# thangvubk/SoftGroup

Measured on AMD Instinct MI355X. Metric: scans/sec ScanNet-v2-like inference (softgroup_scannet.yaml, full forward_test), higher is better.
Workload: dtype f32

## Files before the change

include/softgroup_hip.h:

```cpp
#ifndef SOFTGROUP_HIP_H
#define SOFTGROUP_HIP_H

#include <stddef.h>
#include <stdint.h>

#ifdef __cplusplus
extern "C" {
#endif

typedef void *sg_stream_t;

#define SG_OK 0
#define SG_ERR_ARG (-1)
#define SG_ERR_WORKSPACE (-2)
#define SG_ERR_LAUNCH (-3)
#define SG_ERR_UNSUPPORTED (-4)

#define SG_BALLQUERY_MAX_NEIGHBORS 1000
#define SG_OCTREE_NUM_NODES 585
#define SG_OCTREE_NUM_LEAVES 512
#define SG_LISTS_SORTED 1
#define SG_LISTS_RADIUS 2

int sg_version(void);
const char *sg_last_error(void);
int sg_device_info(char *name_host, int name_cap, int *num_cu_host, int *clock_khz_host);

int sg_stream_release(sg_stream_t stream);
int sg_stream_create(sg_stream_t *stream_out);
int sg_stream_destroy(sg_stream_t stream);
int sg_stream_create_priority(sg_stream_t *stream_out, int level);

int sg_voxelize_idx_host(const int64_t *coords_host, int n, int ncol, int mode,
                         int32_t *input_map_host, int32_t *num_voxels_host,
                         int32_t *max_active_host);
int sg_voxelize_idx_fill_host(const int64_t *coords_host, int n, int ncol, int mode,
                              const int32_t *input_map_host, int num_voxels, int max_active,
                              int64_t *out_coords_host, int32_t *out_map_host);
size_t sg_voxelize_idx_workspace_bytes(int n);
int sg_voxelize_idx_build(const int64_t *coords, int n, int ncol, int mode, int32_t *input_map,
                          int32_t *meta, void *ws, size_t ws_bytes, sg_stream_t stream);
int sg_voxelize_idx_fill(const int64_t *coords, int n, int ncol, int mode,
                         const int32_t *input_map, int num_voxels, int max_active,
                         int64_t *out_coords, int32_t *out_map, void *ws, size_t ws_bytes,
                         sg_stream_t stream);

int sg_voxelize_fp(const float *feats, const int32_t *rules, int num_voxels, int max_active,
                   int channels, int average, float *out, sg_stream_t stream);
int sg_voxelize_bp(const float *d_out, const int32_t *rules, int num_voxels, int max_active,
                   int channels, int average, float *d_feats, sg_stream_t stream);

size_t sg_ballquery_workspace_bytes(int n);
int sg_ballquery_build_grid(const float *xyz, const int32_t *batch_idxs, int n, float radius,
                            void *ws, size_t ws_bytes, sg_stream_t stream);
int sg_ballquery_count(const float *xyz, const int32_t *batch_idxs, int n, float radius,
                       int32_t *start_len, int32_t *meta, void *ws, size_t ws_bytes,
                       sg_stream_t stream);
int sg_ballquery_fill(const float *xyz, const int32_t *batch_idxs, int n, float radius,
                      const int32_t *start_len, int32_t *idx, void *ws, size_t ws_bytes,
                      sg_stream_t stream);
size_t sg_scan_workspace_bytes(int n);
int sg_exclusive_scan_startlen(int32_t *start_len, int n, int32_t *meta, void *ws,
                               size_t ws_bytes, sg_stream_t stream);

int sg_octree_build_host(const float *points_host, const float *xyzwhl_host, int num_points,
                         int num_levels, float *boxes_host, int32_t *pt_inds_host,
                         int32_t *pt_start_len_host);
size_t sg_octree_build_workspace_bytes(int n);
int sg_octree_build(const float *points, int n, float *boxes, int32_t *pt_inds, int32_t *pt_start_len,
                    void *ws, size_t ws_bytes, sg_stream_t stream);
size_t sg_pyramid_inverse_map_workspace_bytes(int n_points, int n_voxels, int n_prop);
int sg_pyramid_inverse_map(const int32_t *proposals_idx, int64_t num_pairs, int n_prop,
                           const int32_t *l2p_map, int n_points, int n_voxels, int32_t *out_idx,
                           int32_t *out_offsets, int32_t *n_out_dev, void *ws, size_t ws_bytes,
                           sg_stream_t stream);
int sg_octree_ballquery_count(const float *points, const float *boxes, const int32_t *pt_inds,
                              const int32_t *pt_start_len, int n, float radius,
                              int32_t *start_len, sg_stream_t stream);
int sg_octree_ballquery_fill(const float *points, const float *boxes, const int32_t *pt_inds,
                             const int32_t *pt_start_len, int n, float radius,
                             const int32_t *start_len, int32_t *idx, sg_stream_t stream);

size_t sg_bfs_workspace_bytes(int n, int64_t n_edges);
// ... 228 lines not shown
  int n_points;
  int n_sem_classes;
  int n_seg;
  const int32_t *seg_class;
  const float *seg_thr;
  float score_thr;
  int min_npoint;
  float radius;
  int batch_size;
  float voxel_scale;
  int voxel_shape;
  int feat_channels;
} sg_grouping_cfg;
typedef struct sg_grouping_result {
  int n_selected, n_neighbours, n_proposals, sum_npoint, n_voxels, max_active;
  size_t proposals_idx;
  size_t proposals_offset;
  size_t voxel_coords;
  size_t voxel_offsets;
  size_t voxel_feats;
  size_t point_to_voxel;
  size_t arena_used, arena_needed;
  int deferred_classes;
  int reserved_;
} sg_grouping_result;
int sg_scan_grouping(const sg_grouping_cfg *cfg, const float *scores, const float *pt_offsets,
                     const float *coords_float, const int32_t *batch_idxs, const float *point_feats,
                     void *arena, size_t arena_bytes, sg_grouping_result *result_host,
                     sg_stream_t stream);

typedef struct sg_grouping_pp_cfg {
  sg_grouping_cfg base;
  int with_pyramid, with_octree, lvl_fusion;
  double radius;
  double base_size;
} sg_grouping_pp_cfg;
int sg_scan_grouping_pp(const sg_grouping_pp_cfg *cfg, const float *scores, const float *pt_offsets,
                        const float *coords_float, const int32_t *batch_idxs, const float *point_feats,
                        void *arena, size_t arena_bytes, sg_grouping_result *result_host,
                        sg_stream_t stream);

int sg_host_copy_2d(void *dst, int64_t dst_pitch_bytes, const void *src, int64_t src_pitch_bytes, int64_t rows,
                    int64_t row_bytes);
int sg_host_cast_f64_f32(float *dst, const double *src, int64_t n);
int sg_host_fill_i64_strided(int64_t *dst, int64_t pitch_elems, int64_t rows, int64_t value);
int sg_host_colmax_i64(const int64_t *src, int64_t rows, int64_t cols, int64_t *out_max);

// ... 231 lines not shown
```

softgroup_amd/_lib.py:

```python
import ctypes as C
import os

_HERE = os.path.dirname(os.path.abspath(__file__))
LIB_PATH = os.path.join(_HERE, 'lib', os.environ.get('SG_LIB_NAME', 'libsoftgroup_hip.so'))

_lib = None

_vp, _i, _f, _i64, _sz = C.c_void_p, C.c_int, C.c_float, C.c_int64, C.c_size_t
_pi32 = C.POINTER(C.c_int32)

SIGNATURES = {
    'sg_version': (_i, []),
    'sg_last_error': (C.c_char_p, []),
    'sg_device_info': (_i, [C.c_char_p, _i, C.POINTER(_i), C.POINTER(_i)]),
    'sg_stream_release': (_i, [_vp]),
    'sg_host_copy_2d': (_i, [_vp, _i64, _vp, _i64, _i64, _i64]),
    'sg_host_cast_f64_f32': (_i, [_vp, _vp, _i64]),
    'sg_host_fill_i64_strided': (_i, [_vp, _i64, _i64, _i64]),
    'sg_host_colmax_i64': (_i, [_vp, _i64, _i64, _vp]),
    'sg_stream_create': (_i, [_vp]),
    'sg_stream_create_priority': (_i, [_vp, _i]),
    'sg_stream_destroy': (_i, [_vp]),
    'sg_voxelize_idx_host': (_i, [_vp, _i, _i, _i, _vp, _pi32, _pi32]),
    'sg_voxelize_idx_fill_host': (_i, [_vp, _i, _i, _i, _vp, _i, _i, _vp, _vp]),
    'sg_voxelize_idx_workspace_bytes': (_sz, [_i]),
    'sg_voxelize_idx_build': (_i, [_vp, _i, _i, _i, _vp, _vp, _vp, _sz, _vp]),
    'sg_voxelize_idx_fill': (_i, [_vp, _i, _i, _i, _vp, _i, _i, _vp, _vp, _vp, _sz, _vp]),
    'sg_voxelize_fp': (_i, [_vp, _vp, _i, _i, _i, _i, _vp, _vp]),
    'sg_voxelize_bp': (_i, [_vp, _vp, _i, _i, _i, _i, _vp, _vp]),
    'sg_ballquery_workspace_bytes': (_sz, [_i]),
    'sg_ballquery_build_grid': (_i, [_vp, _vp, _i, _f, _vp, _sz, _vp]),
    'sg_ballquery_count': (_i, [_vp, _vp, _i, _f, _vp, _vp, _vp, _sz, _vp]),
    'sg_ballquery_fill': (_i, [_vp, _vp, _i, _f, _vp, _vp, _vp, _sz, _vp]),
    'sg_scan_workspace_bytes': (_sz, [_i]),
    'sg_exclusive_scan_startlen': (_i, [_vp, _i, _vp, _vp, _sz, _vp]),
    'sg_octree_build_host': (_i, [_vp, _vp, _i, _i, _vp, _vp, _vp]),
    'sg_octree_build_workspace_bytes': (_sz, [_i]),
    'sg_octree_build': (_i, [_vp, _i, _vp, _vp, _vp, _vp, _sz, _vp]),
    'sg_pyramid_inverse_map_workspace_bytes': (_sz, [_i, _i, _i]),
    'sg_pyramid_inverse_map': (_i, [_vp, _i64, _i, _vp, _i, _i, _vp, _vp, _vp, _vp, _sz, _vp]),
    'sg_octree_ballquery_count': (_i, [_vp, _vp, _vp, _vp, _i, _f, _vp, _vp]),
    'sg_octree_ballquery_fill': (_i, [_vp, _vp, _vp, _vp, _i, _f, _vp, _vp, _vp]),
    'sg_bfs_workspace_bytes': (_sz, [_i, _i64]),
    'sg_bfs_cluster_label': (_i, [_vp, _vp, _i, _i64, _i, _vp, _vp, _i, _pi32, _pi32, _vp, _sz, _vp]),
    'sg_bfs_cluster_emit': (_i, [_vp, _vp, _i, _i64, _vp, _vp, _i, _i, _vp, _vp, _vp, _sz, _vp]),
    'sg_sec_mean': (_i, [_vp, _vp, _i, _i, _vp, _vp]),
    'sg_sec_min': (_i, [_vp, _vp, _i, _i, _vp, _vp]),
    'sg_sec_max': (_i, [_vp, _vp, _i, _i, _vp, _vp]),
    'sg_global_avg_pool_fp': (_i, [_vp, _vp, _i, _i, _vp, _vp]),
    'sg_global_avg_pool_bp': (_i, [_vp, _vp, _vp, _i, _i, _vp]),
    'sg_get_mask_iou_on_cluster': (_i, [_vp, _vp, _vp, _vp, _i, _i, _vp, _vp]),
    'sg_get_mask_iou_on_pred': (_i, [_vp, _vp, _vp, _vp, _vp, _i, _i, _vp, _vp]),
    'sg_get_mask_label': (_i, [_vp, _vp, _vp, _vp, _vp, _i, _i, _f, _vp, _vp]),
    'sg_spconv_hash_workspace_bytes': (_sz, [_i]),
    'sg_spconv_subm_rulebook': (_i, [_vp, _i, _pi32, _vp, _vp, _sz, _vp]),
    'sg_spconv_pyramid_workspace_bytes': (_sz, [_i, _i]),
# ... 160 lines not shown
```

softgroup_amd/csrc/ballquery.hip:

```cpp
#include "common.h"
#include "scan.h"

namespace sg {

constexpr int32_t kBqEmpty = 0x7f7f7f7f;
constexpr int kBqBuf = 2048;
constexpr int kBqCap = SG_BALLQUERY_MAX_NEIGHBORS;
constexpr int kBqKeep = 64;

struct BqWs {
  int4 *cell;
  int32_t *table;
  int32_t *count;
  int32_t *start;
  int32_t *cursor;
  int32_t *slot_of;
  float4 *sorted;
  int32_t *keep;
  void *scan_ws;
  size_t scan_bytes;
  uint32_t cap;
};

__device__ __forceinline__ uint32_t cell_slot(int b, int cx, int cy, int cz, uint32_t mask) {
  uint64_t h = (static_cast<uint64_t>(static_cast<uint32_t>(b)) << 32) | static_cast<uint32_t>(cx);
  h = mix64(h) ^ ((static_cast<uint64_t>(static_cast<uint32_t>(cy)) << 32) | static_cast<uint32_t>(cz));
  return static_cast<uint32_t>(mix64(h)) & mask;
}

__global__ void __launch_bounds__(256) bq_insert_kernel(const float *__restrict__ xyz,
                                                       const int32_t *__restrict__ batch_idxs,
                                                       int n, double inv_cell, int4 *__restrict__ cell,
                                                       int32_t *table, uint32_t mask, int32_t *count,
                                                       int32_t *__restrict__ slot_of) {
  const int i = blockIdx.x * 256 + threadIdx.x;
  if (i >= n) return;
  int4 c;
  c.x = batch_idxs ? batch_idxs[i] : 0;
  c.y = static_cast<int>(floor(static_cast<double>(xyz[3 * i + 0]) * inv_cell));
  c.z = static_cast<int>(floor(static_cast<double>(xyz[3 * i + 1]) * inv_cell));
  c.w = static_cast<int>(floor(static_cast<double>(xyz[3 * i + 2]) * inv_cell));
// ... 53 lines not shown
    lo = right ? mid + 1 : lo;
    hi = right ? hi : mid;
  }
  return __shfl(c.start, lo, 64) + (t - __shfl(c.excl, lo, 64));
}

__device__ __forceinline__ int bq_scan_count(const float4 *__restrict__ sorted, const BqCells &c,
                                             float ox, float oy, float oz, float r2, int limit) {
  int total = 0;
  for (int t0 = 0; t0 < c.total; t0 += 64) {
    const int t = t0 + lane_id();
    const int at = bq_candidate(c, min(t, c.total - 1));
    if (t < c.total) {
      const float4 p = sorted[at];
      total += (dist2(ox, oy, oz, p.x, p.y, p.z) < r2 && __float_as_int(p.w) < limit) ? 1 : 0;
    }
  }
  return wave_sum(total);
}

template <bool FILL>
__global__ void __launch_bounds__(256) bq_query_kernel(const float *__restrict__ xyz, int n,
                                                      float r2, const int4 *__restrict__ cell,
                                                      const int32_t *__restrict__ table,
                                                      const int32_t *__restrict__ count,
                                                      const int32_t *__restrict__ start,
                                                      uint32_t mask, const float4 *__restrict__ sorted,
                                                      int32_t *__restrict__ start_len,
                                                      int32_t *__restrict__ idx_out, int32_t *__restrict__ keep) {
  __shared__ __attribute__((aligned(16))) int32_t buf_all[FILL ? 4 * kBqBuf : 4 * kBqKeep];
  const int wave = threadIdx.x >> 6, lane = threadIdx.x & 63;
  int32_t *buf = buf_all + wave * (FILL ? kBqBuf : kBqKeep);
  for (int i = blockIdx.x * 4 + wave; i < n; i += gridDim.x * 4) {
    if (FILL) {
      const int out_len = start_len[2 * i + 1];
      if (out_len <= kBqKeep) {
        if (lane < out_len) idx_out[static_cast<int64_t>(start_len[2 * i]) + lane] = keep[static_cast<int64_t>(i) * kBqKeep + lane];
        continue;
      }
    }
    const float ox = xyz[3 * i], oy = xyz[3 * i + 1], oz = xyz[3 * i + 2];
    const int4 c = cell[i];
    int my_start = 0, my_count = 0;
    if (lane < 27) {
      const int cx = c.y + lane / 9 - 1, cy = c.z + (lane / 3) % 3 - 1, cz = c.w + lane % 3 - 1;
      uint32_t s = cell_slot(c.x, cx, cy, cz, mask);
      while (true) {
        const int32_t rep = table[s];
        if (rep == kBqEmpty) break;
        const int4 o = cell[rep];
        if (o.x == c.x && o.y == cx && o.z == cy && o.w == cz) {
          my_start = start[s];
          my_count = count[s];
          break;
        }
        s = (s + 1) & mask;
      }
    }
    const BqCells cells = bq_cells(my_start, my_count);
    if (!FILL) {
      int m = 0;
      for (int t0 = 0; t0 < cells.total; t0 += 64) {
        const int t = t0 + lane;
        const int at = bq_candidate(cells, min(t, cells.total - 1));
        bool ok = false;
        int id = 0;
        if (t < cells.total) {
          const float4 p = sorted[at];
          id = __float_as_int(p.w);
          ok = dist2(ox, oy, oz, p.x, p.y, p.z) < r2;
        }
        const uint64_t bal = __ballot(ok);
        const int pos = m + mask_prefix(bal);
        if (ok && pos < kBqKeep) buf[pos] = id;
        m += __popcll(bal);
      }
      if (lane == 0) start_len[2 * i + 1] = min(m, kBqCap);
      if (m <= kBqKeep) {
        __builtin_amdgcn_fence(__ATOMIC_RELEASE, "wavefront");
        __builtin_amdgcn_wave_barrier();
        const int e = lane < m ? buf[lane] : 0x7fffffff;
        int rank = 0;
        for (int j = 0; j < m; ++j) rank += (buf[j] < e);
        if (lane < m) keep[static_cast<int64_t>(i) * kBqKeep + rank] = e;
      }
      __builtin_amdgcn_wave_barrier();
      continue;
    }
    const int out_start = start_len[2 * i], out_len = start_len[2 * i + 1];
    int limit = 0x7fffffff;
    int m = 0;
    for (int attempt = 0; attempt < 2; ++attempt) {
      m = 0;
      for (int t0 = 0; t0 < cells.total; t0 += 64) {
        const int t = t0 + lane;
        const int at = bq_candidate(cells, min(t, cells.total - 1));
        bool ok = false;
        int id = 0;
        if (t < cells.total) {
          const float4 p = sorted[at];
// ... 10 lines not shown
      while (lo < hi) {
        const int mid = lo + (hi - lo) / 2;
        const int cmid = bq_scan_count(sorted, cells, ox, oy, oz, r2, mid);
        if (cmid >= out_len) hi = mid; else lo = mid + 1;
      }
      limit = lo;
    }
    __builtin_amdgcn_fence(__ATOMIC_RELEASE, "wavefront");
    __builtin_amdgcn_wave_barrier();
    for (int e0 = 0; e0 < m; e0 += 64) {
      const int ei = e0 + lane;
      const int e = ei < m ? buf[ei] : 0x7fffffff;
      int rank = 0;
      int j = 0;
      for (; j + 4 <= m; j += 4) {
        const int4 q = *reinterpret_cast<const int4 *>(buf + j);
        rank += (q.x < e) + (q.y < e) + (q.z < e) + (q.w < e);
      }
      for (; j < m; ++j) rank += (buf[j] < e);
      if (ei < m && rank < out_len) idx_out[static_cast<int64_t>(out_start) + rank] = e;
    }
    __builtin_amdgcn_wave_barrier();
  }
}

static size_t bq_cap(int n) {
  size_t cap = 1024;
  while (cap < static_cast<size_t>(n) * 2) cap <<= 1;
  return cap;
}

static bool bq_carve(void *ws, size_t ws_bytes, int n, BqWs *w) {
  Workspace a(ws, ws_bytes);
  const size_t nn = static_cast<size_t>(n > 0 ? n : 1);
  w->cap = static_cast<uint32_t>(bq_cap(n));
  w->cell = a.take<int4>(nn);
  w->sorted = a.take<float4>(nn);
  w->table = a.take<int32_t>(w->cap);
  w->count = a.take<int32_t>(w->cap);
  w->start = a.take<int32_t>(w->cap);
  w->cursor = a.take<int32_t>(w->cap);
  w->slot_of = a.take<int32_t>(nn);
  w->scan_bytes = scan_workspace_bytes(w->cap);
  w->scan_ws = a.take<char>(w->scan_bytes);
  w->keep = a.take<int32_t>(nn * kBqKeep);
  return w->scan_ws != nullptr && w->keep != nullptr;
}

}

using namespace sg;

extern "C" {

size_t sg_ballquery_workspace_bytes(int n) {
  const size_t nn = static_cast<size_t>(n > 0 ? n : 1);
  const size_t cap = bq_cap(n);
  return 2 * align_up(nn * 16) + 4 * align_up(cap * 4) + align_up(nn * 4) +
         align_up(scan_workspace_bytes(cap)) + align_up(nn * kBqKeep * 4) + 256;
}

int sg_ballquery_build_grid(const float *xyz, const int32_t *batch_idxs, int n, float radius,
                            void *ws, size_t ws_bytes, sg_stream_t stream_) {
  SG_REQUIRE(n >= 0 && radius > 0.f, "sg_ballquery_build_grid: bad arguments (n=%d r=%g)", n, radius);
  hipStream_t stream = as_stream(stream_);
  BqWs w;
  if (!bq_carve(ws, ws_bytes, n, &w)) {
    set_error("sg_ballquery_build_grid: workspace too small");
    return SG_ERR_WORKSPACE;
  }
  if (n == 0) return SG_OK;
  {
    FillList f;
    f.add(w.table, static_cast<size_t>(w.cap) * 4, 0x7f);
    f.add(w.count, static_cast<size_t>(w.cap) * 4, 0);
    f.add(w.cursor, static_cast<size_t>(w.cap) * 4, 0);
    fill_many(f, stream);
  }
  const double inv_cell = 1.0 / (static_cast<double>(radius) * (1.0 + 1e-6));
  const int grid = (n + 255) / 256;
  bq_insert_kernel<<<grid, 256, 0, stream>>>(xyz, batch_idxs, n, inv_cell, w.cell, w.table,
                                             w.cap - 1, w.count, w.slot_of);
  const int32_t *count = w.count;
  int32_t *start = w.start;
  auto in = [count] __device__(int64_t s) { return count[s]; };
  auto out = [start] __device__(int64_t s, int v) { start[s] = v; };
  int rc = exclusive_scan(in, out, w.cap, nullptr, w.scan_ws, w.scan_bytes, stream);
  if (rc != SG_OK) return rc;
  bq_scatter_kernel<<<grid, 256, 0, stream>>>(xyz, n, w.slot_of, w.start, w.cursor, w.sorted);
  return check_launch("sg_ballquery_build_grid");
}

int sg_ballquery_count(const float *xyz, const int32_t *batch_idxs, int n, float radius,
                       int32_t *start_len, int32_t *meta, void *ws, size_t ws_bytes,
                       sg_stream_t stream_) {
  (void)batch_idxs;
  (void)meta;
  SG_REQUIRE(n >= 0 && radius > 0.f, "sg_ballquery_count: bad arguments");
  BqWs w;
  if (!bq_carve(ws, ws_bytes, n, &w)) {
    set_error("sg_ballquery_count: workspace too small");
    return SG_ERR_WORKSPACE;
  }
  if (n == 0) return SG_OK;
  const float r2 = radius * radius;
  bq_query_kernel<false><<<grid_for(n, 4, 256 * 16), 256, 0, as_stream(stream_)>>>(
      xyz, n, r2, w.cell, w.table, w.count, w.start, w.cap - 1, w.sorted, start_len, nullptr, w.keep);
  return check_launch("sg_ballquery_count");
}

int sg_ballquery_fill(const float *xyz, const int32_t *batch_idxs, int n, float radius,
                      const int32_t *start_len, int32_t *idx, void *ws, size_t ws_bytes,
                      sg_stream_t stream_) {
  (void)batch_idxs;
  SG_REQUIRE(n >= 0 && radius > 0.f, "sg_ballquery_fill: bad arguments");
  BqWs w;
  if (!bq_carve(ws, ws_bytes, n, &w)) {
    set_error("sg_ballquery_fill: workspace too small");
    return SG_ERR_WORKSPACE;
  }
  if (n == 0) return SG_OK;
  const float r2 = radius * radius;
  bq_query_kernel<true><<<grid_for(n, 4, 256 * 16), 256, 0, as_stream(stream_)>>>(
      xyz, n, r2, w.cell, w.table, w.count, w.start, w.cap - 1, w.sorted,
      const_cast<int32_t *>(start_len), idx, w.keep);
  return check_launch("sg_ballquery_fill");
}

}
```

softgroup_amd/csrc/bfs.hip:

```cpp
#include <stdlib.h>

#include <map>
#include <mutex>
#include <utility>

#include "common.h"
#include "scan.h"

namespace sg {

constexpr int kCap = SG_BALLQUERY_MAX_NEIGHBORS;
constexpr int kEmitThreads = 512;
constexpr int kEmitWaves = kEmitThreads / 64;

#define SG_LD(p) __hip_atomic_load((p), __ATOMIC_RELAXED, __HIP_MEMORY_SCOPE_AGENT)
#define SG_ST(p, v) __hip_atomic_store((p), (v), __ATOMIC_RELAXED, __HIP_MEMORY_SCOPE_AGENT)

struct BfsWs {
  int32_t *parent, *lab, *size, *cid, *coff, *owner, *seeds, *ebase, *wcnt, *asym_nodes;
  int4 *label;
  int2 *erec;
  int32_t *counters;
  void *scan_ws;
  size_t scan_bytes;
// ... 75 lines not shown
  int lo = 0, hi = len;
  while (lo < hi) {
    const int mid = (lo + hi) >> 1;
    const int v = lst[mid];
    if (v < key) lo = mid + 1; else hi = mid;
  }
  return lo < len && lst[lo] == key;
}

__global__ void __launch_bounds__(256) bfs_init_kernel(int n, int32_t *parent, int32_t *size,
                                                      int32_t *owner) {
  const int i = blockIdx.x * 256 + threadIdx.x;
  if (i < n) {
    parent[i] = i;
    size[i] = 0;
    owner[i] = 0x7fffffff;
  }
}

constexpr int kSample = 2;
template <int SAMPLE>
__global__ void __launch_bounds__(256) bfs_union_kernel(const int32_t *__restrict__ idx,
                                                       const int32_t *__restrict__ start_len, int n,
                                                       int lists_sorted, int radius_lists,
                                                       int32_t *parent, int32_t *asym_nodes,
                                                       int32_t *counters) {
  const int wave = threadIdx.x >> 6, lane = threadIdx.x & 63;
  for (int u = blockIdx.x * 4 + wave; u < n; u += gridDim.x * 4) {
    const int st = start_len[2 * u], ln_all = start_len[2 * u + 1];
    const int ln = SAMPLE ? min(ln_all, kSample) : ln_all;
    const bool u_capped = ln_all >= kCap;
    bool any_asym = false;
    const int ru = SAMPLE ? -1 : SG_LD(&parent[u]);
    for (int p0 = 0; p0 < ln; p0 += 64) {
      const int p = p0 + lane;
      const int v = p < ln ? idx[st + p] : u;
      bool sym = true;
      if (v != u) {
        const int vst = start_len[2 * v], vln = start_len[2 * v + 1];
        if (!radius_lists || u_capped || vln >= kCap) {
          if (lists_sorted) {
            sym = list_has_sorted(idx + vst, vln, u);
          } else {
            sym = false;
            for (int j = 0; j < vln; ++j)
              if (idx[vst + j] == u) { sym = true; break; }
          }
        }
        if (sym) {
          if (v < u && (SAMPLE || SG_LD(&parent[v]) != ru)) uf_union(parent, uf_find(parent, u), uf_find(parent, v));
        }
      }
      any_asym |= !sym;
    }
    if (!SAMPLE && __any(any_asym)) {
      if (lane == 0) asym_nodes[atomicAdd(&counters[0], 1)] = u;
    }
  }
}

__global__ void __launch_bounds__(256) bfs_hook_min_kernel(const int32_t *__restrict__ idx,
                                                          const int32_t *__restrict__ start_len, int n,
                                                          int lists_sorted, int radius_lists, int32_t *parent) {
  const int u = blockIdx.x * 256 + threadIdx.x;
  if (u >= n) return;
  const int st = start_len[2 * u], ln = start_len[2 * u + 1];
  if (ln == 0 || !lists_sorted) return;
  const int v = idx[st];
  if (v >= u) return;
  if (!radius_lists || ln >= kCap || start_len[2 * v + 1] >= kCap)
    if (!list_has_sorted(idx + start_len[2 * v], start_len[2 * v + 1], u)) return;
  parent[u] = v;
}
__global__ void __launch_bounds__(256) bfs_compress_kernel(int n, int32_t *parent) {
  const int i = blockIdx.x * 256 + threadIdx.x;
  if (i < n) SG_ST(&parent[i], uf_find(parent, i));
}

__global__ void __launch_bounds__(256) bfs_flatten_kernel(int n, int32_t *parent, int32_t *lab) {
  const int i = blockIdx.x * 256 + threadIdx.x;
  if (i >= n) return;
  int r = i;
  while (true) {
    const int p = SG_LD(&parent[r]);
    if (p == r) break;
    r = p;
  }
  lab[i] = r;
}
__global__ void __launch_bounds__(256) bfs_store_root_kernel(int n, const int32_t *__restrict__ lab,
                                                            int32_t *__restrict__ parent) {
  const int i = blockIdx.x * 256 + threadIdx.x;
  if (i < n) parent[i] = lab[i];
// ... 1442 lines not shown
  const size_t ne = static_cast<size_t>(n_edges > 0 ? n_edges : 1);
  const size_t be = big_stage_entries(n);
  return 14 * align_up(nn * 4) + align_up(64 * 4) + align_up(scan_workspace_bytes(n)) +
         align_up(ne * sizeof(int2)) + 2 * (align_up(be * 4) + align_up(be * 8)) + 256;
}

int sg_bfs_cluster_label(const int32_t *bq_idxs, const int32_t *start_len, int n, int64_t n_edges,
                         int list_flags, const int32_t *seg_of_point, const float *seg_thr,
                         int n_seg, int32_t *n_cluster_host, int32_t *sum_npoint_host, void *ws,
                         size_t ws_bytes, sg_stream_t stream_) {
  SG_REQUIRE(n >= 0 && n_seg >= 1 && seg_thr != nullptr, "sg_bfs_cluster_label: bad arguments");
  hipStream_t stream = as_stream(stream_);
  BfsWs w;
  if (!bfs_carve(ws, ws_bytes, n, n_edges, &w)) {
    set_error("sg_bfs_cluster_label: workspace too small");
    return SG_ERR_WORKSPACE;
  }
  *n_cluster_host = 0;
  *sum_npoint_host = 0;
  if (n == 0) return SG_OK;
  const int grid = (n + 255) / 256;
  hipMemsetAsync(w.counters, 0, 64 * 4, stream);
  bfs_init_kernel<<<grid, 256, 0, stream>>>(n, w.parent, w.size, w.owner);
  static const bool one_pass = getenv("SG_BFS_ONE_PASS") != nullptr;
  if (!one_pass) {
    static const bool sample_env = getenv("SG_BFS_SAMPLE") != nullptr;
    if (sample_env || !(list_flags & SG_LISTS_SORTED))
      bfs_union_kernel<1><<<grid_for(n, 4, 256 * 16), 256, 0, stream>>>(bq_idxs, start_len, n,
                                                                      list_flags & SG_LISTS_SORTED,
                                                                      list_flags & SG_LISTS_RADIUS,
                                                                      w.parent, w.asym_nodes, w.counters);
    else
      bfs_hook_min_kernel<<<grid, 256, 0, stream>>>(bq_idxs, start_len, n, list_flags & SG_LISTS_SORTED,
                                                   list_flags & SG_LISTS_RADIUS, w.parent);
    bfs_compress_kernel<<<grid, 256, 0, stream>>>(n, w.parent);
  }
  bfs_union_kernel<0><<<grid_for(n, 4, 256 * 16), 256, 0, stream>>>(bq_idxs, start_len, n,
                                                                  list_flags & SG_LISTS_SORTED,
                                                                  list_flags & SG_LISTS_RADIUS,
                                                                  w.parent, w.asym_nodes, w.counters);
  bfs_flatten_kernel<<<grid, 256, 0, stream>>>(n, w.parent, w.lab);
  bfs_store_root_kernel<<<grid, 256, 0, stream>>>(n, w.lab, w.parent);

  int32_t *host_counters = pinned_words();
  SG_REQUIRE(host_counters != nullptr, "sg_bfs_cluster_label: pinned allocation failed");
  for (int i = 0; i < 5; ++i) host_counters[i] = 0;
  for (int pass = 0; pass < 2; ++pass) {
    if (pass == 1) {
      const int n_asym = host_counters[0];
      while (true) {
        hipMemsetAsync(w.counters + 1, 0, 4, stream);
        bfs_propagate_kernel<<<grid_for(n_asym, 4, 256 * 16), 256, 0, stream>>>(
            bq_idxs, start_len, w.asym_nodes, n_asym, w.parent, w.lab, w.counters);
        host_counters[8] = 0;
        hipMemcpyAsync(host_counters + 8, w.counters + 1, 4, hipMemcpyDeviceToHost, stream);
        if (hipStreamSynchronize(stream) != hipSuccess) return check_launch("bfs propagate");
        if (!host_counters[8]) break;
      }
      bfs_zero_size_kernel<<<grid, 256, 0, stream>>>(n, w.size);
    }
    bfs_label_kernel<<<grid, 256, 0, stream>>>(n, w.parent, w.lab, start_len, w.label, w.size);
    const int4 *label = w.label;
// ... 190 lines not shown
```

softgroup_amd/csrc/scan_exec.hip:

```cpp
#include <stdlib.h>
#include <string.h>

#include "common.h"
#include "scan.h"

namespace sg {

constexpr int kSelBlock = 256;
constexpr int kMaxSeg = 32;

__global__ void __launch_bounds__(kSelBlock) select_count_kernel(const float *__restrict__ scores, int n,
                                                                int n_cls, const int32_t *__restrict__ seg_class,
                                                                int n_seg, float thr, int n_blocks,
                                                                int32_t *__restrict__ blk_cnt) {
  __shared__ int part[4][kMaxSeg];
  const int i = blockIdx.x * kSelBlock + threadIdx.x;
  const int wave = threadIdx.x >> 6, lane = threadIdx.x & 63;
  for (int s = 0; s < n_seg; ++s) {
    const bool on = i < n && scores[static_cast<int64_t>(i) * n_cls + seg_class[s]] > thr;
    const int c = __popcll(__ballot(on));
    if (lane == 0) part[wave][s] = c;
  }
  __syncthreads();
  if (threadIdx.x < n_seg)
// ... 476 lines not shown
  if (n == 0 || n_seg == 0) return SG_OK;

  const int n_blocks = (n + kSelBlock - 1) / kSelBlock;
  SG_TAKE(meta, int32_t, 64);
  SG_TAKE(blk_cnt, int32_t, static_cast<size_t>(n_seg) * n_blocks);
  SG_TAKE(blk_off, int32_t, static_cast<size_t>(n_seg) * n_blocks);
  select_count_kernel<<<n_blocks, kSelBlock, 0, stream>>>(scores, n, cfg->n_sem_classes, cfg->seg_class, n_seg,
                                                         cfg->score_thr, n_blocks, blk_cnt);
  select_scan_kernel<<<1, 1024, 0, stream>>>(blk_cnt, n_seg, n_blocks, cfg->min_npoint, blk_off, meta);
  SG_TRY(check_launch(kWhat));
  SG_TRY(read_back(host, meta, 1, stream, kWhat));
  const int n_sel = host[0];
  res->n_selected = n_sel;
  if (n_sel == 0) return SG_OK;
  SG_TAKE(obj, int32_t, n_sel);
  SG_TAKE(seg_of, int32_t, n_sel);
  SG_TAKE(pts, float, 3 * static_cast<size_t>(n_sel));
  SG_TAKE(key, int32_t, n_sel);
  select_emit_kernel<<<n_blocks, kSelBlock, 0, stream>>>(scores, n, cfg->n_sem_classes, cfg->seg_class, n_seg,
                                                        cfg->score_thr, n_blocks, blk_off, coords_float,
                                                        pt_offsets, batch_idxs, cfg->batch_size, obj, seg_of,
                                                        pts, key);

  const size_t bq_bytes = sg_ballquery_workspace_bytes(n_sel);
  SG_TAKE(bq_ws, char, bq_bytes);
  SG_TAKE(start_len, int32_t, 2 * static_cast<size_t>(n_sel));
  const size_t sc_bytes = sg_scan_workspace_bytes(n_sel);
  SG_TAKE(sc_ws, char, sc_bytes);
  hipMemsetAsync(start_len, 0, sizeof(int32_t) * 2 * n_sel, stream);
  SG_TRY(sg_ballquery_build_grid(pts, key, n_sel, cfg->radius, bq_ws, bq_bytes, stream_));
  SG_TRY(sg_ballquery_count(pts, key, n_sel, cfg->radius, start_len, nullptr, bq_ws, bq_bytes, stream_));
  SG_TRY(sg_exclusive_scan_startlen(start_len, n_sel, meta + 32, sc_ws, sc_bytes, stream_));
  SG_TRY(read_back(host, meta + 32, 1, stream, kWhat));
  const int n_active = host[0];
  res->n_neighbours = n_active;
  SG_TAKE(bq_idx, int32_t, n_active);
  SG_TRY(sg_ballquery_fill(pts, key, n_sel, cfg->radius, start_len, bq_idx, bq_ws, bq_bytes, stream_));

  const size_t bfs_bytes = sg_bfs_workspace_bytes(n_sel, n_active);
  SG_TAKE(bfs_ws, char, bfs_bytes);
  int32_t n_prop = 0, S = 0;
  SG_TRY(sg_bfs_cluster_label(bq_idx, start_len, n_sel, n_active, SG_LISTS_SORTED | SG_LISTS_RADIUS, seg_of,
                              cfg->seg_thr, n_seg, &n_prop, &S, bfs_ws, bfs_bytes, stream_));
  res->n_proposals = n_prop;
  res->sum_npoint = S;
  if (S == 0) return SG_OK;
  SG_TAKE(pairs, int32_t, 2 * static_cast<size_t>(S));
  SG_TAKE(poff, int32_t, static_cast<size_t>(n_prop) + 1);
  hipMemsetAsync(poff, 0, sizeof(int32_t) * (n_prop + 1), stream);
  if (t_scan_emit_hook != nullptr) t_scan_emit_hook(t_scan_emit_ctx);
  SG_TRY(sg_bfs_cluster_emit(bq_idx, start_len, n_sel, n_active, seg_of, cfg->seg_thr, n_prop, S, pairs, poff,
                             bfs_ws, bfs_bytes, stream_));
  proposal_map_kernel<<<grid_for(S, 256), 256, 0, stream>>>(pairs, S, obj);
  res->proposals_idx = ar.at(pairs);
  res->proposals_offset = ar.at(poff);
  if (cfg->voxel_shape == 0) {
    res->arena_used = ar.off;
    return check_launch(kWhat);
  }

  return voxelise_proposals(cfg, pairs, poff, n_prop, S, coords_float, point_feats, ar, meta, host, res, stream_, kWhat);
}

int sg_scan_grouping_pp(const sg_grouping_pp_cfg *pcfg, const float *scores, const float *pt_offsets,
                        const float *coords_float, const int32_t *batch_idxs, const float *point_feats,
                        void *arena, size_t arena_bytes, sg_grouping_result *res, sg_stream_t stream_) {
  static const char *kWhat = "sg_scan_grouping_pp";
  SG_REQUIRE(pcfg != nullptr && res != nullptr, "sg_scan_grouping_pp: null descriptor");
  const sg_grouping_cfg *cfg = &pcfg->base;
  SG_REQUIRE(cfg->n_points >= 0 && cfg->n_sem_classes >= 1 && cfg->n_seg >= 0 && cfg->n_seg <= kMaxSeg &&
                 cfg->batch_size >= 1 && cfg->feat_channels >= 1 && cfg->voxel_shape >= 0,
             "sg_scan_grouping_pp: bad configuration (n_seg must be <= %d)", kMaxSeg);
  SG_REQUIRE(pcfg->radius > 0 && (!pcfg->with_pyramid || pcfg->base_size > 0),
             "sg_scan_grouping_pp: radius and pyramid_base_size must be positive");
// ... 286 lines not shown
```

softgroup_amd/csrc/scan_forward.hip:

```cpp
#include <stdlib.h>
#include <string.h>
#include <condition_variable>

#include <map>
#include <mutex>
#include <utility>

#include "common.h"
#include "heads.h"

#define SG_TRY_(expr)             \
  do {                            \
    const int rc_ = (expr);       \
    if (rc_ != SG_OK) return rc_; \
  } while (0)

namespace sg {

extern thread_local void (*t_scan_emit_hook)(void *);
extern thread_local void (*t_unet_conv_hook)(void *);
extern thread_local void *t_unet_conv_ctx;
extern thread_local void *t_scan_emit_ctx;

__global__ void __launch_bounds__(256) voxelize_cat_kernel(const float *__restrict__ a, int ca,
// ... 292 lines not shown
  if (rows == 0) return SG_OK;
  const int grid = static_cast<int>((rows + 255) / 256);
  if (channels == 32) mlp_rows_kernel<32><<<grid, 256, 0, as_stream(stream)>>>(feats, idx, rows, as_mlp(*mlp), out);
  else mlp_rows_kernel<16><<<grid, 256, 0, as_stream(stream)>>>(feats, idx, rows, as_mlp(*mlp), out);
  return check_launch("sg_mlp_rows");
}

int sg_linear_rows(const float *x, int64_t rows, const sg_linear *lin, float *out, sg_stream_t stream) {
  SG_REQUIRE(rows >= 0 && lin && lin->w && lin->out >= 1 && lin->in >= 1 && x && out, "sg_linear_rows: bad arguments");
  if (rows == 0) return SG_OK;
  linear_rows_kernel<<<grid_for(rows * lin->out, 256), 256, 0, as_stream(stream)>>>(x, rows, lin->w, lin->b, lin->out,
                                                                                  lin->in, out);
  return check_launch("sg_linear_rows");
}

size_t sg_scan_arena_bytes(const sg_scan_desc *d, int n_points, int n_voxels) {
  if (d == nullptr || d->backbone == nullptr) return 0;
  const size_t N = static_cast<size_t>(n_points > 0 ? n_points : 1), M = static_cast<size_t>(n_voxels > 0 ? n_voxels : 1);
  const size_t C = static_cast<size_t>(d->channels), ns = static_cast<size_t>(d->semantic_classes);
  size_t p = align_up(M * 16) + align_up(M * 8 * 4) + align_up(M * C * 4) + align_up(N * C * 4) + 2 * align_up(N * ns * 4) +
             align_up(N * 12) + 2 * align_up(N * 8) + align_up(N * 96) + (1 << 20);
  size_t bb = sg_unet_arena_bytes(d->backbone, n_voxels) / 4;
  if (bb < (64u << 20)) bb = 64u << 20;
  const size_t later = (160u << 20) + N * 256;
  return p + (bb > later ? bb : later) + (8 << 20);
}

int sg_scan_forward(const sg_scan_desc *d, const sg_scan_input *in, void *arena, size_t arena_bytes, void *host_dense,
                    size_t host_dense_bytes, void *host_inst, size_t host_inst_bytes, sg_scan_result *res,
                    sg_stream_t stream_) {
  static const char *kWhat = "sg_scan_forward";
  SG_REQUIRE(d && in && res && d->backbone, "sg_scan_forward: null descriptor");
  SG_REQUIRE(!d->want_instances || d->tiny, "sg_scan_forward: instances need the tiny U-Net's descriptor");
  SG_REQUIRE(d->channels == 16 || d->channels == 32, "sg_scan_forward: backbone channels must be 16 or 32");
  SG_REQUIRE(d->semantic.out == d->semantic_classes && d->semantic_classes >= 1 && d->semantic_classes <= 32,
             "sg_scan_forward: 1..32 semantic classes");
  SG_REQUIRE(in->n_points >= 0 && in->n_voxels >= 0 && in->max_active >= 0 && in->batch_size >= 1 && in->feat_dim >= 1,
             "sg_scan_forward: bad input sizes");
  SG_REQUIRE(in->n_dense >= 0 && in->n_dense <= SG_SCAN_DENSE_MAX, "sg_scan_forward: at most %d dense items",
             SG_SCAN_DENSE_MAX);
  memset(res, 0, sizeof(*res));
  hipStream_t stream = as_stream(stream_);
  const int N = in->n_points, M = in->n_voxels, C = d->channels, ns = d->semantic_classes;
  const int cin = in->feat_dim + (d->with_coords ? 3 : 0);
  SG_REQUIRE(d->backbone->input_w == nullptr ? cin == C : cin == d->backbone->input_cin,
             "sg_scan_forward: %d feature columns, the backbone takes %d", cin,
             d->backbone->input_w ? d->backbone->input_cin : C);
// ... 272 lines not shown
```

softgroup_amd/model/native_scan.py:

```python
import ctypes as C
import threading

import numpy as np
import torch

from .. import _lib as L

_ERR_WORKSPACE = -2


class GroupingCfg(C.Structure):
    _fields_ = [('n_points', C.c_int), ('n_sem_classes', C.c_int), ('n_seg', C.c_int),
                ('seg_class', C.c_void_p), ('seg_thr', C.c_void_p), ('score_thr', C.c_float),
                ('min_npoint', C.c_int), ('radius', C.c_float), ('batch_size', C.c_int),
                ('voxel_scale', C.c_float), ('voxel_shape', C.c_int), ('feat_channels', C.c_int)]


class GroupingPPCfg(C.Structure):
    _fields_ = [('base', GroupingCfg), ('with_pyramid', C.c_int), ('with_octree', C.c_int), ('lvl_fusion', C.c_int),
                ('radius', C.c_double), ('base_size', C.c_double)]


class GroupingResult(C.Structure):
    _fields_ = [('n_selected', C.c_int), ('n_neighbours', C.c_int), ('n_proposals', C.c_int),
                ('sum_npoint', C.c_int), ('n_voxels', C.c_int), ('max_active', C.c_int),
                ('proposals_idx', C.c_size_t), ('proposals_offset', C.c_size_t),
                ('voxel_coords', C.c_size_t), ('voxel_offsets', C.c_size_t),
                ('voxel_feats', C.c_size_t), ('point_to_voxel', C.c_size_t),
                ('arena_used', C.c_size_t), ('arena_needed', C.c_size_t),
                ('deferred_classes', C.c_int), ('reserved_', C.c_int)]


class InstancesCfg(C.Structure):
    _fields_ = [('n_proposals', C.c_int), ('n_classes', C.c_int), ('score_stride', C.c_int),
                ('sum_npoint', C.c_int64), ('n_points', C.c_int), ('cls_score_thr', C.c_float),
                ('mask_score_thr', C.c_float), ('min_npoint', C.c_int)]


class InstancesResult(C.Structure):
    _fields_ = [('n_kept', C.c_int), ('off_class', C.c_size_t), ('off_score', C.c_size_t),
                ('off_text', C.c_size_t), ('text_bytes', C.c_size_t), ('host_needed', C.c_size_t),
                ('arena_used', C.c_size_t), ('arena_needed', C.c_size_t),
                ('bits', C.c_size_t), ('label_id', C.c_size_t)]


_arenas = {}
_host = threading.local()


def _arena(tag, nbytes, device):
    key = (tag, device, L.stream())
    t = _arenas.get(key)
    if t is None or t.numel() < nbytes:
# ... 102 lines not shown
```

Baseline: 405.9.

## Keep short ball-query lists in place and skip scan-plus-fill for them

```diff
diff --git a/include/softgroup_hip.h b/include/softgroup_hip.h
--- a/include/softgroup_hip.h
+++ b/include/softgroup_hip.h
@@ -21,6 +21,7 @@
 #define SG_OCTREE_NUM_LEAVES 512
 #define SG_LISTS_SORTED 1
 #define SG_LISTS_RADIUS 2
+#define SG_LISTS_UNCAPPED 4
 
 int sg_version(void);
 const char *sg_last_error(void);
@@ -59,6 +60,13 @@
 int sg_ballquery_fill(const float *xyz, const int32_t *batch_idxs, int n, float radius,
                       const int32_t *start_len, int32_t *idx, void *ws, size_t ws_bytes,
                       sg_stream_t stream);
+int sg_ballquery_count_lists(const float *xyz, const int32_t *batch_idxs, int n, float radius,
+                             int32_t *start_len, int32_t *stats, void *ws, size_t ws_bytes,
+                             sg_stream_t stream);
+const int32_t *sg_ballquery_lists_base(void *ws, size_t ws_bytes, int n);
+int sg_ballquery_fill_long(const float *xyz, const int32_t *batch_idxs, int n, float radius,
+                           int32_t *start_len, int32_t *overflow, int64_t n_long, void *ws,
+                           size_t ws_bytes, int64_t *span, sg_stream_t stream);
 size_t sg_scan_workspace_bytes(int n);
 int sg_exclusive_scan_startlen(int32_t *start_len, int n, int32_t *meta, void *ws,
                                size_t ws_bytes, sg_stream_t stream);
@@ -333,7 +341,7 @@
   size_t point_to_voxel;
   size_t arena_used, arena_needed;
   int deferred_classes;
-  int reserved_;
+  int list_form;
 } sg_grouping_result;
 int sg_scan_grouping(const sg_grouping_cfg *cfg, const float *scores, const float *pt_offsets,
                      const float *coords_float, const int32_t *batch_idxs, const float *point_feats,
diff --git a/softgroup_amd/_lib.py b/softgroup_amd/_lib.py
--- a/softgroup_amd/_lib.py
+++ b/softgroup_amd/_lib.py
@@ -32,6 +32,9 @@
     'sg_ballquery_build_grid': (_i, [_vp, _vp, _i, _f, _vp, _sz, _vp]),
     'sg_ballquery_count': (_i, [_vp, _vp, _i, _f, _vp, _vp, _vp, _sz, _vp]),
     'sg_ballquery_fill': (_i, [_vp, _vp, _i, _f, _vp, _vp, _vp, _sz, _vp]),
+    'sg_ballquery_count_lists': (_i, [_vp, _vp, _i, _f, _vp, _vp, _vp, _sz, _vp]),
+    'sg_ballquery_lists_base': (_vp, [_vp, _sz, _i]),
+    'sg_ballquery_fill_long': (_i, [_vp, _vp, _i, _f, _vp, _vp, _i64, _vp, _sz, C.POINTER(C.c_int64), _vp]),
     'sg_scan_workspace_bytes': (_sz, [_i]),
     'sg_exclusive_scan_startlen': (_i, [_vp, _i, _vp, _vp, _sz, _vp]),
     'sg_octree_build_host': (_i, [_vp, _vp, _i, _i, _vp, _vp, _vp]),
diff --git a/softgroup_amd/csrc/ballquery.hip b/softgroup_amd/csrc/ballquery.hip
--- a/softgroup_amd/csrc/ballquery.hip
+++ b/softgroup_amd/csrc/ballquery.hip
@@ -7,6 +7,12 @@
 constexpr int kBqBuf = 2048;
 constexpr int kBqCap = SG_BALLQUERY_MAX_NEIGHBORS;
 constexpr int kBqKeep = 64;
+
+struct __attribute__((aligned(32))) BqSlot {
+  int4 key;
+  int start, count, pad0, pad1;
+};
+static_assert(sizeof(BqSlot) == 32, "one probe = one 32-byte record");
 
 struct BqWs {
   int4 *cell;
@@ -17,6 +23,7 @@
   int32_t *slot_of;
   float4 *sorted;
   int32_t *keep;
+  struct BqSlot *slot;
   void *scan_ws;
   size_t scan_bytes;
   uint32_t cap;
@@ -116,20 +123,22 @@
 template <bool FILL>
 __global__ void __launch_bounds__(256) bq_query_kernel(const float *__restrict__ xyz, int n,
                                                       float r2, const int4 *__restrict__ cell,
-                                                      const int32_t *__restrict__ table,
-                                                      const int32_t *__restrict__ count,
-                                                      const int32_t *__restrict__ start,
+                                                      const BqSlot *__restrict__ slot,
                                                       uint32_t mask, const float4 *__restrict__ sorted,
                                                       int32_t *__restrict__ start_len,
-                                                      int32_t *__restrict__ idx_out, int32_t *__restrict__ keep) {
+                                                      int32_t *__restrict__ idx_out, int32_t *keep,
+                                                      int32_t *stats) {
   __shared__ __attribute__((aligned(16))) int32_t buf_all[FILL ? 4 * kBqBuf : 4 * kBqKeep];
+  __shared__ int32_t wave_stats[4][3];
   const int wave = threadIdx.x >> 6, lane = threadIdx.x & 63;
   int32_t *buf = buf_all + wave * (FILL ? kBqBuf : kBqKeep);
+  int sum_pairs = 0, sum_long = 0, max_len = 0;
   for (int i = blockIdx.x * 4 + wave; i < n; i += gridDim.x * 4) {
     if (FILL) {
       const int out_len = start_len[2 * i + 1];
       if (out_len <= kBqKeep) {
-        if (lane < out_len) idx_out[static_cast<int64_t>(start_len[2 * i]) + lane] = keep[static_cast<int64_t>(i) * kBqKeep + lane];
+        if (keep != nullptr && lane < out_len)
+          idx_out[static_cast<int64_t>(start_len[2 * i]) + lane] = keep[static_cast<int64_t>(i) * kBqKeep + lane];
         continue;
       }
     }
@@ -140,12 +149,12 @@
       const int cx = c.y + lane / 9 - 1, cy = c.z + (lane / 3) % 3 - 1, cz = c.w + lane % 3 - 1;
       uint32_t s = cell_slot(c.x, cx, cy, cz, mask);
       while (true) {
-        const int32_t rep = table[s];
-        if (rep == kBqEmpty) break;
-        const int4 o = cell[rep];
+        const int4 o = slot[s].key;
+        const int2 range = *reinterpret_cast<const int2 *>(&slot[s].start);
+        if (range.y == 0) break;
         if (o.x == c.x && o.y == cx && o.z == cy && o.w == cz) {
-          my_start = start[s];
-          my_count = count[s];
+          my_start = range.x;
+          my_count = range.y;
           break;
         }
         s = (s + 1) & mask;
@@ -169,7 +178,18 @@
         if (ok && pos < kBqKeep) buf[pos] = id;
         m += __popcll(bal);
       }
-      if (lane == 0) start_len[2 * i + 1] = min(m, kBqCap);
+      const int len = min(m, kBqCap);
+      if (stats == nullptr) {
+        if (lane == 0) start_len[2 * i + 1] = len;
+      } else {
+        if (lane == 0) {
+          if (m <= kBqKeep) *reinterpret_cast<int2 *>(start_len + 2 * i) = make_int2(i * kBqKeep, len);
+          else start_len[2 * i + 1] = len;
+        }
+        sum_pairs += len;
+        sum_long += m > kBqKeep ? len : 0;
+        max_len = max(max_len, len);
+      }
       if (m <= kBqKeep) {
         __builtin_amdgcn_fence(__ATOMIC_RELEASE, "wavefront");
         __builtin_amdgcn_wave_barrier();
@@ -226,6 +246,20 @@
     }
     __builtin_amdgcn_wave_barrier();
   }
+  if (!FILL && stats != nullptr) {
+    if (lane == 0) {
+      wave_stats[wave][0] = sum_pairs;
+      wave_stats[wave][1] = sum_long;
+      wave_stats[wave][2] = max_len;
+    }
+    __syncthreads();
+    if (threadIdx.x < 3) {
+      const int a = wave_stats[0][threadIdx.x], b = wave_stats[1][threadIdx.x], c = wave_stats[2][threadIdx.x],
+                d = wave_stats[3][threadIdx.x];
+      if (threadIdx.x == 2) atomicMax(&stats[2], max(max(a, b), max(c, d)));
+      else if (a + b + c + d != 0) atomicAdd(&stats[threadIdx.x], a + b + c + d);
+    }
+  }
 }
 
 static size_t bq_cap(int n) {
@@ -247,8 +281,9 @@
   w->slot_of = a.take<int32_t>(nn);
   w->scan_bytes = scan_workspace_bytes(w->cap);
   w->scan_ws = a.take<char>(w->scan_bytes);
+  w->slot = a.take<BqSlot>(w->cap);
   w->keep = a.take<int32_t>(nn * kBqKeep);
-  return w->scan_ws != nullptr && w->keep != nullptr;
+  return w->scan_ws != nullptr && w->slot != nullptr && w->keep != nullptr;
 }
 
 }
@@ -261,7 +296,7 @@
   const size_t nn = static_cast<size_t>(n > 0 ? n : 1);
   const size_t cap = bq_cap(n);
   return 2 * align_up(nn * 16) + 4 * align_up(cap * 4) + align_up(nn * 4) +
-         align_up(scan_workspace_bytes(cap)) + align_up(nn * kBqKeep * 4) + 256;
+         align_up(scan_workspace_bytes(cap)) + align_up(cap * sizeof(BqSlot)) + align_up(nn * kBqKeep * 4) + 256;
 }
 
 int sg_ballquery_build_grid(const float *xyz, const int32_t *batch_idxs, int n, float radius,
@@ -288,7 +323,19 @@
   const int32_t *count = w.count;
   int32_t *start = w.start;
   auto in = [count] __device__(int64_t s) { return count[s]; };
-  auto out = [start] __device__(int64_t s, int v) { start[s] = v; };
+  const int32_t *table = w.table;
+  const int4 *cell = w.cell;
+  BqSlot *slot = w.slot;
+  auto out = [start, count, table, cell, slot] __device__(int64_t s, int v) {
+    start[s] = v;
+    const int32_t rep = table[s];
+    BqSlot r;
+    r.key = rep == kBqEmpty ? make_int4(kBqEmpty, kBqEmpty, kBqEmpty, kBqEmpty) : cell[rep];
+    r.start = v;
+    r.count = rep == kBqEmpty ? 0 : count[s];
+    r.pad0 = r.pad1 = 0;
+    slot[s] = r;
+  };
   int rc = exclusive_scan(in, out, w.cap, nullptr, w.scan_ws, w.scan_bytes, stream);
   if (rc != SG_OK) return rc;
   bq_scatter_kernel<<<grid, 256, 0, stream>>>(xyz, n, w.slot_of, w.start, w.cursor, w.sorted);
@@ -309,8 +356,65 @@
   if (n == 0) return SG_OK;
   const float r2 = radius * radius;
   bq_query_kernel<false><<<grid_for(n, 4, 256 * 16), 256, 0, as_stream(stream_)>>>(
-      xyz, n, r2, w.cell, w.table, w.count, w.start, w.cap - 1, w.sorted, start_len, nullptr, w.keep);
+      xyz, n, r2, w.cell, w.slot, w.cap - 1, w.sorted, start_len, nullptr, w.keep, nullptr);
   return check_launch("sg_ballquery_count");
+}
+
+int sg_ballquery_count_lists(const float *xyz, const int32_t *batch_idxs, int n, float radius,
+                             int32_t *start_len, int32_t *stats, void *ws, size_t ws_bytes,
+                             sg_stream_t stream_) {
+  (void)batch_idxs;
+  SG_REQUIRE(n >= 0 && radius > 0.f && stats != nullptr, "sg_ballquery_count_lists: bad arguments");
+  SG_REQUIRE(static_cast<int64_t>(n) * kBqKeep < 0x7fffffffLL, "sg_ballquery_count_lists: %d points: list starts leave 31 bits", n);
+  BqWs w;
+  if (!bq_carve(ws, ws_bytes, n, &w)) {
+    set_error("sg_ballquery_count_lists: workspace too small");
+    return SG_ERR_WORKSPACE;
+  }
+  hipMemsetAsync(stats, 0, 3 * sizeof(int32_t), as_stream(stream_));
+  if (n == 0) return SG_OK;
+  const float r2 = radius * radius;
+  bq_query_kernel<false><<<grid_for(n, 4, 256 * 16), 256, 0, as_stream(stream_)>>>(
+      xyz, n, r2, w.cell, w.slot, w.cap - 1, w.sorted, start_len, nullptr, w.keep, stats);
+  return check_launch("sg_ballquery_count_lists");
+}
+
+const int32_t *sg_ballquery_lists_base(void *ws, size_t ws_bytes, int n) {
+  BqWs w;
+  return bq_carve(ws, ws_bytes, n, &w) ? w.keep : nullptr;
+}
+
+int sg_ballquery_fill_long(const float *xyz, const int32_t *batch_idxs, int n, float radius,
+                           int32_t *start_len, int32_t *overflow, int64_t n_long, void *ws,
+                           size_t ws_bytes, int64_t *span, sg_stream_t stream_) {
+  (void)batch_idxs;
+  SG_REQUIRE(n >= 0 && radius > 0.f && n_long >= 0 && span != nullptr, "sg_ballquery_fill_long: bad arguments");
+  BqWs w;
+  if (!bq_carve(ws, ws_bytes, n, &w)) {
+    set_error("sg_ballquery_fill_long: workspace too small");
+    return SG_ERR_WORKSPACE;
+  }
+  *span = static_cast<int64_t>(n) * kBqKeep;
+  if (n == 0 || n_long == 0) return SG_OK;
+  SG_REQUIRE(overflow != nullptr && overflow >= w.keep + static_cast<int64_t>(n) * kBqKeep,
+             "sg_ballquery_fill_long: the overflow block must lie behind the workspace");
+  const int64_t first = overflow - w.keep;
+  SG_REQUIRE(first + n_long < 0x7fffffffLL, "sg_ballquery_fill_long: the overflow block is %lld entries from the lists' base: starts leave 31 bits",
+             static_cast<long long>(first));
+  *span = first + n_long;
+  hipStream_t stream = as_stream(stream_);
+  const int32_t *sl = start_len;
+  const int base = static_cast<int>(first);
+  auto in = [sl] __device__(int64_t i) { const int m = sl[2 * i + 1]; return m > kBqKeep ? m : 0; };
+  auto out = [start_len, base] __device__(int64_t i, int v) {
+    if (start_len[2 * i + 1] > kBqKeep) start_len[2 * i] = base + v;
+  };
+  int rc = exclusive_scan(in, out, n, nullptr, w.scan_ws, w.scan_bytes, stream);
+  if (rc != SG_OK) return rc;
+  const float r2 = radius * radius;
+  bq_query_kernel<true><<<grid_for(n, 4, 256 * 16), 256, 0, stream>>>(
+      xyz, n, r2, w.cell, w.slot, w.cap - 1, w.sorted, start_len, w.keep, nullptr, nullptr);
+  return check_launch("sg_ballquery_fill_long");
 }
 
 int sg_ballquery_fill(const float *xyz, const int32_t *batch_idxs, int n, float radius,
@@ -326,8 +430,7 @@
   if (n == 0) return SG_OK;
   const float r2 = radius * radius;
   bq_query_kernel<true><<<grid_for(n, 4, 256 * 16), 256, 0, as_stream(stream_)>>>(
-      xyz, n, r2, w.cell, w.table, w.count, w.start, w.cap - 1, w.sorted,
-      const_cast<int32_t *>(start_len), idx, w.keep);
+      xyz, n, r2, w.cell, w.slot, w.cap - 1, w.sorted, const_cast<int32_t *>(start_len), idx, w.keep, nullptr);
   return check_launch("sg_ballquery_fill");
 }
 
diff --git a/softgroup_amd/csrc/bfs.hip b/softgroup_amd/csrc/bfs.hip
--- a/softgroup_amd/csrc/bfs.hip
+++ b/softgroup_amd/csrc/bfs.hip
@@ -121,7 +121,7 @@
 template <int SAMPLE>
 __global__ void __launch_bounds__(256) bfs_union_kernel(const int32_t *__restrict__ idx,
                                                        const int32_t *__restrict__ start_len, int n,
-                                                       int lists_sorted, int radius_lists,
+                                                       int lists_sorted, int radius_lists, int all_sym,
                                                        int32_t *parent, int32_t *asym_nodes,
                                                        int32_t *counters) {
   const int wave = threadIdx.x >> 6, lane = threadIdx.x & 63;
@@ -135,7 +135,9 @@
       const int p = p0 + lane;
       const int v = p < ln ? idx[st + p] : u;
       bool sym = true;
-      if (v != u) {
+      if (all_sym) {
+        if (v < u && (SAMPLE || SG_LD(&parent[v]) != ru)) uf_union(parent, uf_find(parent, u), uf_find(parent, v));
+      } else if (v != u) {
         const int vst = start_len[2 * v], vln = start_len[2 * v + 1];
         if (!radius_lists || u_capped || vln >= kCap) {
           if (lists_sorted) {
@@ -160,14 +162,15 @@
 
 __global__ void __launch_bounds__(256) bfs_hook_min_kernel(const int32_t *__restrict__ idx,
                                                           const int32_t *__restrict__ start_len, int n,
-                                                          int lists_sorted, int radius_lists, int32_t *parent) {
+                                                          int lists_sorted, int radius_lists, int all_sym,
+                                                          int32_t *parent) {
   const int u = blockIdx.x * 256 + threadIdx.x;
   if (u >= n) return;
   const int st = start_len[2 * u], ln = start_len[2 * u + 1];
   if (ln == 0 || !lists_sorted) return;
   const int v = idx[st];
   if (v >= u) return;
-  if (!radius_lists || ln >= kCap || start_len[2 * v + 1] >= kCap)
+  if (!all_sym && (!radius_lists || ln >= kCap || start_len[2 * v + 1] >= kCap))
     if (!list_has_sorted(idx + start_len[2 * v], start_len[2 * v + 1], u)) return;
   parent[u] = v;
 }
@@ -1656,22 +1659,23 @@
   const int grid = (n + 255) / 256;
   hipMemsetAsync(w.counters, 0, 64 * 4, stream);
   bfs_init_kernel<<<grid, 256, 0, stream>>>(n, w.parent, w.size, w.owner);
+  const int all_sym = (list_flags & SG_LISTS_RADIUS) && (list_flags & SG_LISTS_UNCAPPED) ? 1 : 0;
   static const bool one_pass = getenv("SG_BFS_ONE_PASS") != nullptr;
   if (!one_pass) {
     static const bool sample_env = getenv("SG_BFS_SAMPLE") != nullptr;
     if (sample_env || !(list_flags & SG_LISTS_SORTED))
       bfs_union_kernel<1><<<grid_for(n, 4, 256 * 16), 256, 0, stream>>>(bq_idxs, start_len, n,
                                                                       list_flags & SG_LISTS_SORTED,
-                                                                      list_flags & SG_LISTS_RADIUS,
+                                                                      list_flags & SG_LISTS_RADIUS, all_sym,
                                                                       w.parent, w.asym_nodes, w.counters);
     else
       bfs_hook_min_kernel<<<grid, 256, 0, stream>>>(bq_idxs, start_len, n, list_flags & SG_LISTS_SORTED,
-                                                   list_flags & SG_LISTS_RADIUS, w.parent);
+                                                   list_flags & SG_LISTS_RADIUS, all_sym, w.parent);
     bfs_compress_kernel<<<grid, 256, 0, stream>>>(n, w.parent);
   }
   bfs_union_kernel<0><<<grid_for(n, 4, 256 * 16), 256, 0, stream>>>(bq_idxs, start_len, n,
                                                                   list_flags & SG_LISTS_SORTED,
-                                                                  list_flags & SG_LISTS_RADIUS,
+                                                                  list_flags & SG_LISTS_RADIUS, all_sym,
                                                                   w.parent, w.asym_nodes, w.counters);
   bfs_flatten_kernel<<<grid, 256, 0, stream>>>(n, w.parent, w.lab);
   bfs_store_root_kernel<<<grid, 256, 0, stream>>>(n, w.lab, w.parent);
diff --git a/softgroup_amd/csrc/scan_exec.hip b/softgroup_amd/csrc/scan_exec.hip
--- a/softgroup_amd/csrc/scan_exec.hip
+++ b/softgroup_amd/csrc/scan_exec.hip
@@ -522,26 +522,53 @@
                                                         pt_offsets, batch_idxs, cfg->batch_size, obj, seg_of,
                                                         pts, key);
 
-  const size_t bq_bytes = sg_ballquery_workspace_bytes(n_sel);
-  SG_TAKE(bq_ws, char, bq_bytes);
   SG_TAKE(start_len, int32_t, 2 * static_cast<size_t>(n_sel));
   const size_t sc_bytes = sg_scan_workspace_bytes(n_sel);
   SG_TAKE(sc_ws, char, sc_bytes);
+  const size_t bq_bytes = sg_ballquery_workspace_bytes(n_sel);
+  SG_TAKE(bq_ws, char, bq_bytes);
   hipMemsetAsync(start_len, 0, sizeof(int32_t) * 2 * n_sel, stream);
   SG_TRY(sg_ballquery_build_grid(pts, key, n_sel, cfg->radius, bq_ws, bq_bytes, stream_));
-  SG_TRY(sg_ballquery_count(pts, key, n_sel, cfg->radius, start_len, nullptr, bq_ws, bq_bytes, stream_));
-  SG_TRY(sg_exclusive_scan_startlen(start_len, n_sel, meta + 32, sc_ws, sc_bytes, stream_));
-  SG_TRY(read_back(host, meta + 32, 1, stream, kWhat));
-  const int n_active = host[0];
-  res->n_neighbours = n_active;
-  SG_TAKE(bq_idx, int32_t, n_active);
-  SG_TRY(sg_ballquery_fill(pts, key, n_sel, cfg->radius, start_len, bq_idx, bq_ws, bq_bytes, stream_));
-
-  const size_t bfs_bytes = sg_bfs_workspace_bytes(n_sel, n_active);
+  bool in_place = !(getenv("SG_GROUP_INPLACE") && atoi(getenv("SG_GROUP_INPLACE")) == 0) &&
+                  static_cast<int64_t>(n_sel) * 64 < (1LL << 30);
+  if (in_place) {
+    const size_t need = sg_bfs_workspace_bytes(n_sel, static_cast<int64_t>(n_sel) * 64) + 8 * static_cast<size_t>(n_sel) + (8u << 20);
+    in_place = ar.cap >= ar.off && ar.cap - ar.off >= need;
+  }
+  const int32_t *bq_idx = nullptr;
+  int64_t span = 0;
+  int list_flags = SG_LISTS_SORTED | SG_LISTS_RADIUS;
+  if (in_place) {
+    SG_TRY(sg_ballquery_count_lists(pts, key, n_sel, cfg->radius, start_len, meta + 32, bq_ws, bq_bytes, stream_));
+    SG_TRY(read_back(host, meta + 32, 3, stream, kWhat));
+    const int n_long = host[1], max_len = host[2];
+    res->n_neighbours = host[0];
+    if (max_len < SG_BALLQUERY_MAX_NEIGHBORS) list_flags |= SG_LISTS_UNCAPPED;
+    int32_t *over = nullptr;
+    if (n_long > 0) {
+      SG_TAKE(over_, int32_t, n_long);
+      over = over_;
+    }
+    SG_TRY(sg_ballquery_fill_long(pts, key, n_sel, cfg->radius, start_len, over, n_long, bq_ws, bq_bytes, &span, stream_));
+    bq_idx = sg_ballquery_lists_base(bq_ws, bq_bytes, n_sel);
+    res->list_form = 1 | (list_flags & SG_LISTS_UNCAPPED ? 2 : 0);
+  } else {
+    SG_TRY(sg_ballquery_count(pts, key, n_sel, cfg->radius, start_len, nullptr, bq_ws, bq_bytes, stream_));
+    SG_TRY(sg_exclusive_scan_startlen(start_len, n_sel, meta + 32, sc_ws, sc_bytes, stream_));
+    SG_TRY(read_back(host, meta + 32, 1, stream, kWhat));
+    const int n_active = host[0];
+    res->n_neighbours = n_active;
+    span = n_active;
+    SG_TAKE(bq_csr, int32_t, n_active);
+    SG_TRY(sg_ballquery_fill(pts, key, n_sel, cfg->radius, start_len, bq_csr, bq_ws, bq_bytes, stream_));
+    bq_idx = bq_csr;
+  }
+
+  const size_t bfs_bytes = sg_bfs_workspace_bytes(n_sel, span);
   SG_TAKE(bfs_ws, char, bfs_bytes);
   int32_t n_prop = 0, S = 0;
-  SG_TRY(sg_bfs_cluster_label(bq_idx, start_len, n_sel, n_active, SG_LISTS_SORTED | SG_LISTS_RADIUS, seg_of,
-                              cfg->seg_thr, n_seg, &n_prop, &S, bfs_ws, bfs_bytes, stream_));
+  SG_TRY(sg_bfs_cluster_label(bq_idx, start_len, n_sel, span, list_flags, seg_of, cfg->seg_thr, n_seg, &n_prop, &S,
+                              bfs_ws, bfs_bytes, stream_));
   res->n_proposals = n_prop;
   res->sum_npoint = S;
   if (S == 0) return SG_OK;
@@ -549,7 +576,7 @@
   SG_TAKE(poff, int32_t, static_cast<size_t>(n_prop) + 1);
   hipMemsetAsync(poff, 0, sizeof(int32_t) * (n_prop + 1), stream);
   if (t_scan_emit_hook != nullptr) t_scan_emit_hook(t_scan_emit_ctx);
-  SG_TRY(sg_bfs_cluster_emit(bq_idx, start_len, n_sel, n_active, seg_of, cfg->seg_thr, n_prop, S, pairs, poff,
+  SG_TRY(sg_bfs_cluster_emit(bq_idx, start_len, n_sel, span, seg_of, cfg->seg_thr, n_prop, S, pairs, poff,
                              bfs_ws, bfs_bytes, stream_));
   proposal_map_kernel<<<grid_for(S, 256), 256, 0, stream>>>(pairs, S, obj);
   res->proposals_idx = ar.at(pairs);
diff --git a/softgroup_amd/csrc/scan_forward.hip b/softgroup_amd/csrc/scan_forward.hip
--- a/softgroup_amd/csrc/scan_forward.hip
+++ b/softgroup_amd/csrc/scan_forward.hip
@@ -338,7 +338,7 @@
              align_up(N * 12) + 2 * align_up(N * 8) + align_up(N * 96) + (1 << 20);
   size_t bb = sg_unet_arena_bytes(d->backbone, n_voxels) / 4;
   if (bb < (64u << 20)) bb = 64u << 20;
-  const size_t later = (160u << 20) + N * 256;
+  const size_t later = (160u << 20) + N * 896;
   return p + (bb > later ? bb : later) + (8 << 20);
 }
 
diff --git a/softgroup_amd/model/native_scan.py b/softgroup_amd/model/native_scan.py
--- a/softgroup_amd/model/native_scan.py
+++ b/softgroup_amd/model/native_scan.py
@@ -28,7 +28,7 @@
                 ('voxel_coords', C.c_size_t), ('voxel_offsets', C.c_size_t),
                 ('voxel_feats', C.c_size_t), ('point_to_voxel', C.c_size_t),
                 ('arena_used', C.c_size_t), ('arena_needed', C.c_size_t),
-                ('deferred_classes', C.c_int), ('reserved_', C.c_int)]
+                ('deferred_classes', C.c_int), ('list_form', C.c_int)]
 
 
 class InstancesCfg(C.Structure):
```

Result: no change. 402.3 (-0.9%).
